# temudschin/xfemm

Hardware: AMD Instinct MI355X
Metric: solved DoF/s (assembly+CG to tol) on 2M-tri magnetostatic (higher is better)
Workload: dtype f64; 1 GPU; configs[2]: synthetic 2000000-tri square-domain magnetostatic, linear mu, tol 1e-08; triangles=2000000, dof_total=1002001, dof_per_gpu=1002001, nnz=7006001, pcg_iters=18, newton_iters=1, pcg=Chronopoulos-Gear + AMG V-cycle, parallelism=single GPU

## Files before the change

### xfemm_amd/csrc/xfk_amg.hip

```cpp
#include <hipcub/hipcub.hpp>

#include <algorithm>
#include <climits>
#include <cmath>
#include <cstdio>
#include <cstdlib>
#include <cstring>
#include <map>
#include <mutex>
#include <vector>

#include "xfk_amg_impl.h"
#include "xfk_comm.h"

namespace xfk {

namespace {



using MisKey = unsigned;
constexpr MisKey kStIn = 2u, kStUnd = 1u;
constexpr MisKey kKeyMask = 0x3FFFFFFFu;

// ... 1253 lines not shown
static int build_col16(hipStream_t st, int n, const int *rowptr, const int *col, long long nnz,
                       DBuf<unsigned short> &c16, DBuf<int> &base)
{
    const int nt = (n + B - 1) / B;
    AMG_CHECK(c16.alloc((size_t)std::max(1LL, nnz)));
    AMG_CHECK(base.alloc((size_t)std::max(1, nt)));
    if (nt > 0) k_tile_col16<B><<<nt, 256, 0, st>>>(n, rowptr, col, c16.p, base.p);
    AMG_CHECK(hipGetLastError());
    return XFK_OK;
}

int Amg::aggregate(hipStream_t s, int l, long long &nc, bool allow_stop)
{
    AmgLevel &A = *L[l];
    const int n = A.n;
    const ColView cv{A.col, A.has16 ? A.a16.p : nullptr, A.has16 ? A.a16b.p : nullptr};
    nc = 0;
    A.nc = 0;
    AMG_CHECK(key.alloc(n));
    AMG_CHECK(t1.alloc(n));
    const std::string lv = g_prof ? "setup L" + std::to_string(l) + " " : std::string();
    if (g_prof) g_prof->begin(lv + "MIS-2 aggregation", 0.0);
    int rounds = 0;
    int *und2 = dev_int.p + 4;
    int *run = dev_int.p + 7;
    AMG_CHECK(act.alloc(n));
    k_mis_init<<<std::max(1, nb(n)), kB, 0, s>>>(n, cnt.p, key.p, und2 + 1, run, act.p);
    AMG_CHECK(flag.alloc((size_t)n + 1));
    AMG_CHECK(cursor.alloc((size_t)n + 1));
    auto hint = mis_hint.find(l);
    const bool spec = !g_prof && !A.dist && hint != mis_hint.end() && cap_hint.count(4 * l) &&
                      def_n + 4 <= kAmgDeferSlots && !env_set("XFK_AMG_DEBUG");
    bool joined = false;
    auto joins_and_p = [&]() { return joins_and_p_impl(s, l); };
    AMG_CHECK(mis_out.alloc(4));
    for (int batch = hint != mis_hint.end() ? std::max(1, hint->second) : 12;; batch = 2) {
        for (int b = 0; b < batch; ++b, ++rounds) {
            int *cur = und2 + (rounds & 1), *prev = und2 + ((rounds + 1) & 1);
            const bool last = b + 1 == batch;
            if (A.nnz > 9LL * n) {
                k_mis_max<4><<<nb(4LL * n), kB, 0, s>>>(n, A.rowptr, cv, sflag.p, key.p, t1.p, prev, cur, run, act.p);
                if (last)
                    k_mis_update<4, true><<<nb(4LL * n), kB, 0, s>>>(n, A.rowptr, cv, sflag.p, t1.p, key.p, prev, cur,
                                                                      flag.p);
                else
                    k_mis_update<4><<<nb(4LL * n), kB, 0, s>>>(n, A.rowptr, cv, sflag.p, t1.p, key.p, prev, cur,
                                                                nullptr);
            } else {
                k_mis_max<1><<<nb(n), kB, 0, s>>>(n, A.rowptr, cv, sflag.p, key.p, t1.p, prev, cur, run, act.p);
                if (last)
                    k_mis_update<1, true><<<nb(n), kB, 0, s>>>(n, A.rowptr, cv, sflag.p, t1.p, key.p, prev, cur,
                                                                flag.p);
                else
                    k_mis_update<1><<<nb(n), kB, 0, s>>>(n, A.rowptr, cv, sflag.p, t1.p, key.p, prev, cur, nullptr);
            }
        }
        int rc = scan_only(*this, s, flag.p, cursor.p, n);
        if (rc != XFK_OK) return rc;
        k_mis_pack<<<1, 64, 0, s>>>(cursor.p + n, und2 + ((rounds - 1) & 1), run, mis_out.p);
        AMG_CHECK(hipMemcpyAsync(host_int + 8, mis_out.p, 3 * sizeof(int), hipMemcpyDeviceToHost, s));
        AMG_CHECK(hipEventRecord(ev_host, s));
        joined = spec;
        if (spec && (rc = joins_and_p()) != XFK_OK) return rc;
        AMG_CHECK(hipEventSynchronize(ev_host));
        if (!host_int[9]) break;
        joined = false;
        if (rounds > 4096) {
            set_error("AMG: MIS-2 aggregation did not terminate");
            return XFK_ERR_NOCONV;
        }
    }
    mis_hint[l] = host_int[10];
    nc = host_int[8];
    stats.mis_rounds[l] = host_int[10];
    int rc = XFK_OK;
    if (allow_stop && (nc == 0 || nc > (long long)(0.9 * n))) {
        nc = 0;
        return XFK_OK;
    }
    if (!joined && (rc = joins_and_p()) != XFK_OK) return rc;
    A.nc = (int)nc;
    if (env_set("XFK_AMG_DEBUG")) std::fprintf(stderr, "[amg] level %d P nnz %lld\n", l, A.pnnz);
    AMG_CHECK(A.rrow.alloc((size_t)nc + 1));
    AMG_CHECK(A.rcol.alloc((size_t)std::max(1LL, A.pnnz)));
    AMG_CHECK(A.rval.alloc((size_t)std::max(1LL, A.pnnz)));
    const bool off = !A.dist && !dist;
    hipStream_t ts = s;
    if (off) {
        if ((rc = sw.init()) != XFK_OK) return rc;
        AMG_CHECK(hipEventRecord(sw.a, s));
        AMG_CHECK(hipStreamWaitEvent(sw.cs, sw.a, 0));
        ts = sw.cs;
        sw_used = true;
    }
    if ((rc = transpose_csr(off ? cnt2 : cnt, off ? cub_tmp2 : cub_tmp, ts, n, (int)nc, A.prow.p, A.pcol.p,
                            A.pval.p, A.rrow.p, A.rcol.p, A.rval.p)) != XFK_OK)
        return rc;
    if (off) {
        AMG_CHECK(hipEventRecord(sw.b, sw.cs));
        rt_pending = true;
    }
    if (l == 0 && A.has16 && (rc = build_col16<256>(ts, (int)nc, A.rrow.p, A.rcol.p, A.pnnz, A.r16, A.r16b)) != XFK_OK)
        return rc;
    if (l == 0 && A.has32 && (rc = to_f32(ts, (int)nc, A.rrow.p, A.pnnz, A.rval.p, A.r32)) != XFK_OK) return rc;
    if (l == 0 && A.has32 && A.dist &&
        ((rc = to_f32(ts, n, A.prow.p, A.pnnz, A.pval.p, A.p32)) != XFK_OK ||
         (rc = build_col16<256>(ts, n, A.prow.p, A.pcol.p, A.pnnz, A.p16, A.p16b)) != XFK_OK))
        return rc;
    if (g_prof) g_prof->end();
    return XFK_OK;
}

int Amg::joins_and_p_impl(hipStream_t s, int l)
{
    AmgLevel &A = *L[l];
    const int n = A.n;
    const ColView cv{A.col, A.has16 ? A.a16.p : nullptr, A.has16 ? A.a16b.p : nullptr};
    const std::string lv = g_prof ? "setup L" + std::to_string(l) + " " : std::string();
    AMG_CHECK(agg1.alloc(n));
    AMG_CHECK(agg.alloc(n));
    const int jg = join_lanes((double)A.nnz / std::max(1, n));
    auto joins = [&](auto g) {
        constexpr int G = decltype(g)::value;
        const int blocks = nb((long long)n * G);
        k_agg_join1<G><<<blocks, kB, 0, s>>>(n, A.rowptr, cv, sflag.p, key.p, cursor.p, agg1.p);
        k_agg_join2<G><<<blocks, kB, 0, s>>>(n, A.rowptr, cv, sflag.p, key.p, agg1.p, agg.p);
        k_agg_join3<G><<<blocks, kB, 0, s>>>(n, A.ncol_lim, A.rowptr, cv, A.val, agg.p, agg1.p);
    };
    if (jg == 8) joins(std::integral_constant<int, 8>{});
    else if (jg == 4) joins(std::integral_constant<int, 4>{});
    else joins(std::integral_constant<int, 1>{});
    std::swap(agg.p, agg1.p);
    std::swap(agg.n, agg1.n);
    if (g_prof) g_prof->end();
    if (env_set("XFK_AMG_DEBUG")) {
        DBuf<int> d;
        AMG_CHECK(d.alloc(3));
        AMG_CHECK(hipMemsetAsync(d.p, 0, 3 * sizeof(int), s));
        k_debug_unagg<<<nb(n), kB, 0, s>>>(n, A.rowptr, A.col, cnt.p, agg.p, d.p);
        int h[3];
        unsigned long long r2[2];
        AMG_CHECK(hipMemcpyAsync(h, d.p, sizeof(h), hipMemcpyDeviceToHost, s));
        AMG_CHECK(hipMemcpyAsync(r2, rho.p + 2 * l, sizeof(r2), hipMemcpyDeviceToHost, s));
        AMG_CHECK(hipStreamSynchronize(s));
        double ra, rf;
        std::memcpy(&ra, &r2[0], 8);
        std::memcpy(&rf, &r2[1], 8);
        std::fprintf(stderr, "[amg] rank %d level %d n %d nnz %lld nc %lld unaggregated: strong %d weak-only %d isolated %d "
                     "rhoA/omega %.4g rhoF %.4g mis_rounds %d\n", dist ? rank : 0, l, n, A.nnz, (long long)host_int[8], h[0], h[1],
                     h[2], ra, rf, host_int[10]);
    }
    SgX XS{A.rowptr, A.col, A.val, A.ncol_lim, sflag.p, dfinv.p, wF.p, cv.c16, cv.cbase};
    SgY YT{nullptr, nullptr, nullptr, agg.p};
    if (g_prof) g_prof->begin(lv + "P = (I - w D^-1 A) P_tent, R = P^T", 0.0);
    return spgemm<true>(*this, s, n, XS, YT, A.prow, A.pcol, A.pval, A.pnnz, 4 * l, !A.dist);
}

int Amg::alloc_vectors()
{
    for (int k = 0; k < nlev; ++k) {
        AmgLevel &A = *L[k];
        const size_t nv = (size_t)std::max(1, std::max(A.n, A.ncol_smooth));
        AMG_CHECK(A.xa.alloc(nv));
        AMG_CHECK(A.xb.alloc(nv));
        AMG_CHECK(A.r.alloc((size_t)std::max(1, A.n)));
        if (k > 0) AMG_CHECK(A.b.alloc((size_t)std::max(1, A.n)));
    }
    return XFK_OK;
}

int Amg::build(hipStream_t s, int l0)
{
    int l = l0;
    for (;; ++l) {
        AmgLevel &A = *L[l];
        const int n = A.n;
        stats.n[l] = n;
        stats.nnz[l] = A.nnz;
        A.nc = 0;
        AMG_CHECK(A.dinv.alloc(n));
        AMG_CHECK(absd.alloc(n));
        AMG_CHECK(dfinv.alloc(n));
        AMG_CHECK(wF.alloc(n));
        AMG_CHECK(cnt.alloc((size_t)n + 1));
        const std::string lv = g_prof ? "setup L" + std::to_string(l) + " " : std::string();
        if (g_prof) g_prof->begin(lv + "diagonal, strength, rho", 0.0);
        k_amg_diag<<<nb(n), kB, 0, s>>>(n, A.rowptr, A.col, A.val, absd.p, A.dinv.p);
        if (n <= dense_max) {
            if (g_prof) g_prof->end();
            dense_coarse = true;
            break;
        }
        A.has16 = l == 0 && !A.dist && !dist && col16 != 0;
        A.has32 = A.has16 && prec32 != 0;
        if (A.has16) {
            int rc0 = build_col16<kCgBlock>(s, n, A.rowptr, A.col, A.nnz, A.a16, A.a16b);
            if (rc0 != XFK_OK) return rc0;
        }
        AMG_CHECK(sflag.alloc((size_t)A.nnz));
        AMG_CHECK(rho_part.alloc(2 * (size_t)nb_str(n)));
        k_amg_strength<<<nb_str(n), kB, 0, s>>>(n, A.ncol_lim, theta_at(l), A.rowptr,
                                                ColView{A.col, A.has16 ? A.a16.p : nullptr, A.has16 ? A.a16b.p : nullptr},
                                                A.val, absd.p, A.dinv.p, sflag.p, cnt.p,
                                                dfinv.p, wF.p, rho_part.p);
        k_max_reduce<<<1, kMaxReduceT, 0, s>>>(nb_str(n), rho_part.p, omega, rho.p + 2 * l);
        if (g_prof) g_prof->end();
        if (trace) {
            int rct = trace_strength(s, l);
            if (rct != XFK_OK) return rct;
        }
        if (l == kAmgMaxLevels - 1) break;
        long long nc = 0;
        int rc = aggregate(s, l, nc, true);
        if (rc != XFK_OK) return rc;
        if (nc == 0) break;
        if (trace && (rc = trace_aggregates(s, l)) != XFK_OK) return rc;
        SgX XA{A.rowptr, A.col, A.val, A.ncol_lim, nullptr, nullptr, nullptr, A.has16 ? A.a16.p : nullptr,
               A.has16 ? A.a16b.p : nullptr};
        SgY YP{A.prow.p, A.pcol.p, A.pval.p, nullptr};
        if (fold_pending) {
            AMG_CHECK(hipStreamWaitEvent(s, sw.c, 0));
            fold_pending = false;
        }
        if (g_prof) g_prof->begin(lv + "SpGEMM A P", 0.0);
        const bool pack = !A.dist && nc < kPackMaxCol && spgemm_pack_on();
        XA.pack = pack;
        rc = spgemm<false>(*this, s, n, XA, YP, A.ftrow, ap_col, ap_val, ap_nnz, 4 * l + 1);
        if (g_prof) g_prof->end();
        if (rc != XFK_OK) return rc;
        if ((int)L.size() <= l + 1) L.emplace_back(new AmgLevel());
        AmgLevel &C = *L[l + 1];
        SgX XR{A.rrow.p, A.rcol.p, A.rval.p, INT_MAX, nullptr, nullptr, nullptr};
        XR.pack = pack;
        SgY YAP{A.ftrow.p, ap_col.p, ap_val.p, nullptr};
        if (rt_pending) {
            AMG_CHECK(hipStreamWaitEvent(s, sw.b, 0));
            rt_pending = false;
        }
        if (g_prof) g_prof->begin(lv + "SpGEMM R (A P)", 0.0);
        rc = spgemm<false>(*this, s, (int)nc, XR, YAP, C.rowptr_o, C.col_o, C.val_o, C.nnz, 4 * l + 2);
        if (g_prof) g_prof->end();
        if (rc != XFK_OK) return rc;
        A.fold = fold_on != 0 && sweeps == 1 && !A.dist;
        A.fold_formed = A.fold;
        if (A.fold) {
            if (g_prof) g_prof->begin(lv + "folded transfer P~ = (I - w D^-1 A) P, R~ = P~^T", 0.0);
            A.fnnz = ap_nnz;
            AMG_CHECK(A.ftrow.alloc((size_t)n + 1));
            AMG_CHECK(A.ftcol.alloc((size_t)std::max(1LL, ap_nnz)));
            AMG_CHECK(A.ftval.alloc((size_t)std::max(1LL, ap_nnz)));
            if (l > 0) {
                AMG_CHECK(A.frrow.alloc((size_t)nc + 1));
                AMG_CHECK(A.frcol.alloc((size_t)std::max(1LL, ap_nnz)));
                AMG_CHECK(A.frval.alloc((size_t)std::max(1LL, ap_nnz)));
            }
            if ((rc = sw.init()) != XFK_OK) return rc;
            AMG_CHECK(hipEventRecord(sw.a, s));
            AMG_CHECK(hipStreamWaitEvent(sw.cs, sw.a, 0));
            hipStream_t fs = sw.cs;
            sw_used = true;
            if (n > 0)
                k_fold_p<<<(int)(((long long)n * kFoldLanes + 255) / 256), 256, 0, fs>>>(
                    n, rho.p + 2 * l, A.dinv.p, A.ftrow.p, ap_col.p, ap_val.p, A.prow.p, A.pcol.p, A.pval.p, A.ftcol.p,
                    A.ftval.p);
            if (l == 0 && A.has16 &&
                (rc = build_col16<kCgBlock>(fs, n, A.ftrow.p, A.ftcol.p, ap_nnz, A.f16, A.f16b)) != XFK_OK)
                return rc;
            if (l == 0 && A.has32 && (rc = to_f32(fs, n, A.ftrow.p, ap_nnz, A.ftval.p, A.f32v)) != XFK_OK) return rc;
            AMG_CHECK(hipEventRecord(sw.c, sw.cs));
            fold_pending = true;
            if (l > 0)
                rc = transpose_csr(cnt2, cub_tmp2, fs, n, (int)nc, A.ftrow.p, A.ftcol.p, A.ftval.p, A.frrow.p,
                                   A.frcol.p, A.frval.p);
            if (rc != XFK_OK) return rc;
            if (def_n > 0 && def_n + 2 <= kAmgDeferSlots) {
                AMG_CHECK(hipMemcpyAsync(def_dev.p + def_n + 1, A.ftrow.p + n, sizeof(int), hipMemcpyDeviceToDevice, s));
                def_target[def_n / 2] = &A.fnnz;
                def_n += 2;
            } else if (def_n > 0) {
                int len = 0;
                AMG_CHECK(hipMemcpyAsync(&len, A.ftrow.p + n, sizeof(int), hipMemcpyDeviceToHost, s));
                AMG_CHECK(hipStreamSynchronize(s));
                A.fnnz = len;
            }
            if (g_prof) g_prof->end();
        }
        C.n = (int)nc;
        C.ncol_lim = (int)nc;
        C.ncol_smooth = (int)nc;
        C.rowptr = C.rowptr_o.p;
        C.col = C.col_o.p;
        C.val = C.val_o.p;
    }
    nlev = l + 1;
    {
        AmgLevel &C = *L[nlev - 1];
        const bool nd_spec = dense_coarse && !g_prof && def_n > 0 && nlev - 1 > l0 &&
                             C.n >= 8 * kBj && nd_key_n == C.n && C.col == C.col_o.p &&
                             (size_t)nd_key_nnz <= C.col_o.n && !env_set("XFK_NO_ND");
        if (nd_spec) {
            AMG_CHECK(mis_out.alloc(4));
            AMG_CHECK(hipMemsetAsync(mis_out.p + 3, 0, sizeof(int), s));
            const int nt = (int)std::max((long long)C.n + 1, nd_key_nnz);
            k_pattern_diff<<<nb(nt), kB, 0, s>>>(C.n, C.rowptr, C.col, nd_key_dev.p, (int)nd_key_nnz, mis_out.p + 3);
            AMG_CHECK(hipMemcpyAsync(host_int + 11, mis_out.p + 3, sizeof(int), hipMemcpyDeviceToHost, s));
        }
// ... 758 lines not shown
```

### xfemm_amd/csrc/xfk_amg_spgemm.hip

```cpp
#include <hipcub/hipcub.hpp>

#include <algorithm>
#include <climits>

#include "xfk_amg_impl.h"

namespace xfk {

namespace {


constexpr int kSgMax = 512;

constexpr int ilog2(int v) { return v <= 1 ? 0 : 1 + ilog2(v >> 1); }

template <bool FILL, bool PMODE, int CAP>
__global__ void __launch_bounds__(64) k_spgemm(int nrows, SgX X, SgY Y, int *__restrict__ cnt_out,
                                               const int *__restrict__ crow, int *__restrict__ ccol,
                                               double *__restrict__ cval, int *overflow)
{
    constexpr int kSgHash = 2 * CAP;
    constexpr int kHashShift = 32 - ilog2(kSgHash);
    __shared__ int hk[kSgHash];
    __shared__ int hr[FILL ? kSgHash : 1];
// ... 57 lines not shown
                    if (f != 0 && Y.agg[k] >= 0) {
                        ys = k;
                        len = 1;
                        xv = (f == 2) ? 1.0 - omega : -omega * dfi * X.val[e];
                    }
                } else {
                    ys = Y.rowptr[k];
                    len = Y.rowptr[k + 1] - ys;
                    xv = X.val[e];
                }
            }
        }
        int incl = len;
#pragma unroll
        for (int off = 1; off < 64; off <<= 1) {
            const int t = __shfl_up(incl, off, 64);
            if (lane >= off) incl += t;
        }
        const int total = __shfl(incl, 63, 64);
        c_off[lane] = incl - len;
        c_ys[lane] = ys;
        c_xv[lane] = xv;
        __syncthreads();
        return total;
    };
    auto product = [&](int p, int &key, double &v) {
        int lo = 0, hi = 63;
        while (lo < hi) {
            const int mid = (lo + hi + 1) >> 1;
            if (c_off[mid] <= p) lo = mid;
            else hi = mid - 1;
        }
        if (PMODE) {
            key = Y.agg[c_ys[lo]];
            v = c_xv[lo];
        } else {
            const int q = c_ys[lo] + (p - c_off[lo]);
            key = Y.col[q];
            if (FILL) v = c_xv[lo] * Y.val[q];
        }
    };

    for (int e0 = xs; e0 < xe; e0 += 64) {
        const int total = stage(e0);
        for (int p = lane; p < total; p += 64) {
            int key;
            double v;
            product(p, key, v);
            insert(key);
        }
        __syncthreads();
    }
    if (!FILL) {
        if (lane == 0) {
            cnt_out[row] = s_cnt;
            if (s_ovf || s_cnt > CAP) atomicOr(overflow, 1);
        }
        return;
    }
    for (int t = lane; t < kSgHash; t += 64)
        if (hk[t] != -1) {
            const int m = atomicAdd(&s_m, 1);
            if (m < CAP) {
                lst[m] = hk[t];
                lslot[m] = t;
            }
        }
    __syncthreads();
    const int cnt = min(s_m, CAP);
    const int cb = crow[row];
    for (int m = lane; m < cnt; m += 64) {
        const int key = lst[m];
        int rank = 0;
        for (int q = 0; q < cnt; ++q) rank += lst[q] < key;
        hr[lslot[m]] = rank;
        ccol[cb + rank] = key;
        acc[rank] = 0.0;
    }
    __syncthreads();
    const int4 *r4 = reinterpret_cast<const int4 *>(s_rank);
    for (int e0 = xs; e0 < xe; e0 += 64) {
        const int total = stage(e0);
        for (int p0 = 0; p0 < total; p0 += 64) {
            const int p = p0 + lane;
            int rank = -1;
            double v = 0.0;
            if (p < total) {
                int key;
                product(p, key, v);
                const int h = lookup(key);
                rank = (h >= 0) ? hr[h] : -1;
            }
            s_rank[lane] = rank;
            s_val[lane] = v;
            __syncthreads();
            if (rank >= 0) {
                bool leader = true;
                double sum = 0.0;
#pragma unroll
                for (int m4 = 0; m4 < 16; ++m4) {
                    const int4 q = r4[m4];
                    const int m = 4 * m4;
                    if (q.x == rank) { leader &= (m < lane) ? false : true; sum += s_val[m]; }
                    if (q.y == rank) { leader &= (m + 1 < lane) ? false : true; sum += s_val[m + 1]; }
                    if (q.z == rank) { leader &= (m + 2 < lane) ? false : true; sum += s_val[m + 2]; }
                    if (q.w == rank) { leader &= (m + 3 < lane) ? false : true; sum += s_val[m + 3]; }
                }
                if (leader) acc[rank] += sum;
            }
            __syncthreads();
        }
    }
    for (int m = lane; m < cnt; m += 64) cval[cb + m] = acc[m];
}

template <bool PMODE>
__global__ void k_spgemm_nprod(int nrows, SgX X, SgY Y, int *__restrict__ nprod)
{
    const int row = blockIdx.x * blockDim.x + threadIdx.x;
    if (row >= nrows) return;
    int c = 0;
    for (int e = X.rowptr[row]; e < X.rowptr[row + 1]; ++e) {
        const int k = X.col[e];
        if (k >= X.col_lim) continue;
        if (PMODE) c += (X.mask[e] != 0 && Y.agg[k] >= 0);
        else c += Y.rowptr[k + 1] - Y.rowptr[k];
    }
    nprod[row] = c;
}


__device__ __forceinline__ void wave_lds_sync()
{
    __builtin_amdgcn_fence(__ATOMIC_RELEASE, "wavefront");
    __builtin_amdgcn_wave_barrier();
    __builtin_amdgcn_fence(__ATOMIC_ACQUIRE, "wavefront");
}

__device__ __forceinline__ unsigned xor_lanes(unsigned w, int lm)
{
    const int x = (int)w;
    switch (lm) {
    case 1: return (unsigned)__builtin_amdgcn_update_dpp(x, x, 0xB1, 0xF, 0xF, false);
    case 2: return (unsigned)__builtin_amdgcn_update_dpp(x, x, 0x4E, 0xF, 0xF, false);
    case 4: {
        const int t = __builtin_amdgcn_update_dpp(x, x, 0x104, 0xF, 0x5, false);
        return (unsigned)__builtin_amdgcn_update_dpp(t, x, 0x114, 0xF, 0xA, false);
    }
    case 8: return (unsigned)__builtin_amdgcn_update_dpp(x, x, 0x128, 0xF, 0xF, false);
    default: return (unsigned)__shfl_xor(x, lm, 64);
    }
}

template <bool PMODE, int G, int CAP, bool PACK = false>
__global__ void __launch_bounds__(64) k_spgemm_sort(int nrows, SgX X, SgY Y, int *__restrict__ cnt_out,
                                                    int *__restrict__ pcol, double *__restrict__ pval, int *ovf,
                                                    int *need, int *__restrict__ slab_n)
{
    constexpr int W = 64 / G;
    constexpr int S = CAP / G;
    static_assert(S >= 1 && S * G == CAP, "CAP must be a multiple of G");
    __shared__ int pk_all[W][CAP];
    __shared__ double pv_all[W][CAP];
    const int g = threadIdx.x / G, l = threadIdx.x % G;
    const int row = blockIdx.x * W + g;
    int *pk = pk_all[g];
    double *pv = pv_all[g];
    const bool live = row < nrows;
    int np = 0;
    if (live) {
        const int xs = X.rowptr[row], xe = X.rowptr[row + 1];
        const ColView xc{X.col, X.c16, X.cbase};
        const int cb = xc.base(row);
        double omega = 0.0, dfi = 0.0;
        if (PMODE) {
            omega = X.wF[row];
            dfi = X.dfinv[row];
        }
        for (int e0 = xs; e0 < xe; e0 += G) {
            const int e = e0 + l;
            int len = 0, ys = 0;
            double xv = 0.0;
            if (e < xe) {
                const int k = xc.at(cb, e);
                if (k < X.col_lim) {
                    if (PMODE) {
                        const unsigned char f = X.mask[e];
                        if (f != 0 && Y.agg[k] >= 0) {
                            ys = Y.agg[k];
                            len = 1;
                            xv = (f == 2) ? 1.0 - omega : -omega * dfi * X.val[e];
                        }
                    } else {
                        ys = Y.rowptr[k];
                        len = Y.rowptr[k + 1] - ys;
                        xv = X.val[e];
                    }
                }
            }
            int incl = len;
#pragma unroll
            for (int off = 1; off < G; off <<= 1) {
                const int t = __shfl_up(incl, off, G);
                if (l >= off) incl += t;
            }
            const int total = __shfl(incl, G - 1, G);
            const int o = np + incl - len;
            if (PMODE) {
                if (len && o < CAP) {
                    pk[o] = ys;
                    pv[o] = xv;
                }
            } else {
                constexpr int U = CAP >= 128 ? 8 : 4;
                int yc[U];
                double yv[U];
#pragma unroll
                for (int q = 0; q < U; ++q)
                    if (q < len) {
                        yc[q] = Y.col[ys + q];
                        yv[q] = Y.val[ys + q];
                    }
#pragma unroll
                for (int q = 0; q < U; ++q)
                    if (q < len && o + q < CAP) {
                        pk[o + q] = yc[q];
                        pv[o + q] = xv * yv[q];
                    }
                for (int q = U; q < len && o + q < CAP; ++q) {
                    pk[o + q] = Y.col[ys + q];
                    pv[o + q] = xv * Y.val[ys + q];
                }
            }
            np += total;
        }
        if (need && np > CAP / 2 && l == 0 && *(volatile int *)need == 0) *need = 1;
        if (np > CAP) {
            if (l == 0) *ovf = 1;
            np = CAP;
        }
    }
    wave_lds_sync();
    int key[S];
    double val[S];
    if constexpr (PACK) {
        constexpr int B = ilog2(CAP);
        unsigned w[S];
#pragma unroll
        for (int s = 0; s < S; ++s) {
            const int v = l * S + s;
            w[s] = v < np ? ((unsigned)pk[v] << B) | (unsigned)v : ~0u;
        }
#pragma unroll
        for (int k = 2; k <= CAP; k <<= 1) {
#pragma unroll
            for (int j = k >> 1; j > 0; j >>= 1) {
                if (j < S) {
#pragma unroll
                    for (int s = 0; s < S; ++s) {
                        const int t = s ^ j;
                        if (t > s) {
                            const bool up = ((l * S + s) & k) == 0;
                            const unsigned a = w[s] >> B, b = w[t] >> B;
                            if ((a > b) == up && a != b) {
                                const unsigned tw = w[s];
                                w[s] = w[t];
                                w[t] = tw;
                            }
                        }
                    }
                } else {
                    const int lm = j / S;
                    const bool lower = (l & lm) == 0;
#pragma unroll
                    for (int s = 0; s < S; ++s) {
                        const unsigned ow = xor_lanes(w[s], lm);
                        const unsigned a = w[s] >> B, b = ow >> B;
                        const bool up = ((l * S + s) & k) == 0;
                        const bool take = (lower == up) ? (b < a) : (b > a);
                        if (take) w[s] = ow;
                    }
                }
            }
        }
#pragma unroll
        for (int s = 0; s < S; ++s) {
            const bool real = w[s] != ~0u;
            key[s] = real ? (int)(w[s] >> B) : INT_MAX;
            val[s] = real ? pv[w[s] & (unsigned)(CAP - 1)] : 0.0;
        }
    } else {
#pragma unroll
        for (int s = 0; s < S; ++s) {
            const int v = l * S + s;
            key[s] = v < np ? pk[v] : INT_MAX;
            val[s] = v < np ? pv[v] : 0.0;
        }
#pragma unroll
        for (int k = 2; k <= CAP; k <<= 1) {
#pragma unroll
            for (int j = k >> 1; j > 0; j >>= 1) {
                if (j < S) {
#pragma unroll
                    for (int s = 0; s < S; ++s) {
                        const int t = s ^ j;
                        if (t > s) {
                            const bool up = ((l * S + s) & k) == 0;
                            if ((key[s] > key[t]) == up && key[s] != key[t]) {
                                const int tk = key[s];
                                key[s] = key[t];
                                key[t] = tk;
                                const double tv = val[s];
                                val[s] = val[t];
                                val[t] = tv;
                            }
                        }
                    }
                } else {
                    const int lm = j / S;
                    const bool lower = (l & lm) == 0;
#pragma unroll
                    for (int s = 0; s < S; ++s) {
                        const int ok = __shfl_xor(key[s], lm, G);
                        const double ov = __shfl_xor(val[s], lm, G);
                        const bool up = ((l * S + s) & k) == 0;
                        const bool take = (lower == up) ? (ok < key[s]) : (ok > key[s]);
                        if (take) {
                            key[s] = ok;
                            val[s] = ov;
                        }
                    }
                }
            }
        }
    }
    const int prev_last = __shfl_up(key[S - 1], 1, G);
    int head[S], nh = 0;
    double run[S];
#pragma unroll
    for (int s = 0; s < S; ++s) {
        const int pk_ = s > 0 ? key[s - 1] : (l > 0 ? prev_last : -1);
        head[s] = (key[s] != INT_MAX && key[s] != pk_) ? 1 : 0;
        run[s] = (s > 0 && !head[s]) ? run[s - 1] + val[s] : val[s];
        nh += head[s];
    }
    int seg_open = 1;
#pragma unroll
    for (int s = 0; s < S; ++s) seg_open &= !head[s];
    double carry = run[S - 1];
    int hpre = nh;
    int open = seg_open;
#pragma unroll
    for (int off = 1; off < G; off <<= 1) {
        const double oc = __shfl_up(carry, off, G);
        const int oo = __shfl_up(open, off, G);
        const int oh = __shfl_up(hpre, off, G);
        if (l >= off) {
            if (open) carry = oc + carry;
            open = open && oo;
            hpre += oh;
        }
    }
    double cin = __shfl_up(carry, 1, G);
    int hin = __shfl_up(hpre, 1, G);
    if (l == 0) {
        cin = 0.0;
        hin = 0;
    }
    const int cnt = __shfl(hpre, G - 1, G);
    int upto = cnt;
#pragma unroll
    for (int off = G; off < 64; off <<= 1) {
        const int t = __shfl_up(upto, off, 64);
        if ((int)threadIdx.x >= off) upto += t;
    }
    if (slab_n && threadIdx.x == 63) slab_n[blockIdx.x] = upto;
    if (!live) return;
    const size_t base = slab_n ? (size_t)blockIdx.x * (W * CAP) + (upto - cnt) : (size_t)row * CAP;
    int h = hin;
#pragma unroll
    for (int s = 0; s < S; ++s) {
        bool lead = true;
#pragma unroll
        for (int q = 0; q <= s; ++q) lead = lead && !head[q];
        const double tot = lead ? cin + run[s] : run[s];
        h += head[s];
        const int nk = s + 1 < S ? key[s + 1] : __shfl_down(key[0], 1, G);
        const bool tail = key[s] != INT_MAX && (nk != key[s] || (s + 1 == S && l == G - 1));
        if (tail) {
            pcol[base + h - 1] = key[s];
            pval[base + h - 1] = tot;
        }
    }
    if (l == 0) cnt_out[row] = cnt;
}

template <int L>
__global__ void k_spgemm_compact(int nrows, int cap, const int *__restrict__ crow, const int *__restrict__ pcol,
                                 const double *__restrict__ pval, int *__restrict__ ccol, double *__restrict__ cval,
                                 int *nnz_out)
{
    const long long t = blockIdx.x * (long long)blockDim.x + threadIdx.x;
    if (t == 0 && nnz_out) *nnz_out = crow[nrows];
    const int row = (int)(t / L), l = (int)(t % L);
    if (row >= nrows) return;
    const int b = crow[row], n = crow[row + 1] - b;
    for (int m = l; m < n; m += L) {
        ccol[b + m] = pcol[(size_t)row * cap + m];
        cval[b + m] = pval[(size_t)row * cap + m];
    }
}

constexpr int kSlabLanes = 16;
__global__ void k_spgemm_compact_slab(int nrows, int nslab, int W, int stride, const int *__restrict__ crow,
                                      const int *__restrict__ slab_n, const int *__restrict__ pcol,
                                      const double *__restrict__ pval, int *__restrict__ ccol,
                                      double *__restrict__ cval, int *nnz_out)
{
    const long long t = blockIdx.x * (long long)blockDim.x + threadIdx.x;
    if (t == 0 && nnz_out) *nnz_out = crow[nrows];
    const int b = (int)(t / kSlabLanes), l = (int)(t % kSlabLanes);
    if (b >= nslab) return;
    const int d = crow[b * W], n = slab_n[b];
    const size_t src = (size_t)b * stride;
    for (int m = l; m < n; m += kSlabLanes) {
        ccol[d + m] = pcol[src + m];
        cval[d + m] = pval[src + m];
    }
}

static bool spgemm_slab_on()
{
    return env_int("XFK_SPGEMM_SLAB", 1) != 0;
}
static int sort_rows_per_wave(int cap) { return cap == 16 ? 16 : cap <= 64 ? 8 : cap == 128 ? 4 : 2; }

void launch_compact(hipStream_t s, int nrows, int cap, const int *crow, const int *slab_n, const int *pc,
                    const double *pv, int *ccol, double *cval, int *nnz_out)
{
    if (slab_n) {
        const int W = sort_rows_per_wave(cap), nslab = (nrows + W - 1) / W;
        k_spgemm_compact_slab<<<(unsigned)(((long long)nslab * kSlabLanes + kB - 1) / kB), kB, 0, s>>>(
            nrows, nslab, W, W * cap, crow, slab_n, pc, pv, ccol, cval, nnz_out);
    } else if (cap <= 16)
        k_spgemm_compact<4><<<(unsigned)(((long long)nrows * 4 + kB - 1) / kB), kB, 0, s>>>(nrows, cap, crow, pc, pv,
                                                                                             ccol, cval, nnz_out);
    else if (cap <= 32)
        k_spgemm_compact<8><<<(unsigned)(((long long)nrows * 8 + kB - 1) / kB), kB, 0, s>>>(nrows, cap, crow, pc, pv,
                                                                                             ccol, cval, nnz_out);
    else
        k_spgemm_compact<16><<<(unsigned)(((long long)nrows * 16 + kB - 1) / kB), kB, 0, s>>>(nrows, cap, crow, pc,
                                                                                               pv, ccol, cval, nnz_out);
}

}

template <bool PMODE>
int spgemm(Amg &M, hipStream_t s, int nrows, const SgX &X, const SgY &Y, DBuf<int> &crow, DBuf<int> &ccol,
           DBuf<double> &cval, long long &cnnz, int key, bool defer)
{
    AMG_CHECK(M.cnt.alloc((size_t)nrows + 1 + ((size_t)nrows + 1) / 2));
    AMG_CHECK(crow.alloc((size_t)nrows + 1));
    int *slab_n = spgemm_slab_on() ? M.cnt.p + nrows + 1 : nullptr;
    int *sovf = M.dev_int.p + 6;
    auto launch_sort = [&](int cap, int *ovf, int *need = nullptr) {
        int *pc = M.pad_col.p;
        double *pv = M.pad_val.p;
        if (nrows > 0) {
#define XFK_SORT(GG, CC, WW)                                                       \
    (X.pack ? k_spgemm_sort<PMODE, GG, CC, !PMODE> : k_spgemm_sort<PMODE, GG, CC>) \
        <<<(nrows + WW - 1) / WW, 64, 0, s>>>(nrows, X, Y, M.cnt.p, pc, pv, ovf, need, slab_n)
            if (cap == 16) XFK_SORT(4, 16, 16);
            else if (cap == 32) XFK_SORT(8, 32, 8);
            else if (cap == 64) XFK_SORT(8, 64, 8);
            else if (cap == 128) XFK_SORT(16, 128, 4);
            else XFK_SORT(32, 256, 2);
#undef XFK_SORT
        }
    };
    auto sort_pass = [&](int cap, bool &overflow) -> int {
        AMG_CHECK(M.pad_col.alloc((size_t)nrows * cap));
        AMG_CHECK(M.pad_val.alloc((size_t)nrows * cap));
        AMG_CHECK(hipMemsetAsync(sovf, 0, sizeof(int), s));
        launch_sort(cap, sovf);
        AMG_CHECK(hipMemcpyAsync(M.host_int + 4, sovf, sizeof(int), hipMemcpyDeviceToHost, s));
        int rc = scan_total(M, s, M.cnt.p, crow.p, nrows, cnnz);
        if (rc != XFK_OK) return rc;
        overflow = M.host_int[4] != 0;
        if (overflow) return XFK_OK;
        AMG_CHECK(ccol.alloc((size_t)std::max(1LL, cnnz)));
        AMG_CHECK(cval.alloc((size_t)std::max(1LL, cnnz)));
        if (nrows > 0)
            launch_compact(s, nrows, cap, crow.p, slab_n, M.pad_col.p, M.pad_val.p, ccol.p, cval.p, nullptr);
        return XFK_OK;
    };
    auto deferred_pass = [&](int cap, bool verify = false) -> int {
        int *slot = M.def_dev.p + M.def_n;
        int *need = (verify && cap > 16) ? M.def_dev.p + kAmgDeferSlots + M.def_n / 2 : nullptr;
        M.def_verify[M.def_n / 2] = need ? cap : 0;
        AMG_CHECK(M.pad_col.alloc((size_t)nrows * cap));
        AMG_CHECK(M.pad_val.alloc((size_t)nrows * cap));
        AMG_CHECK(ccol.alloc((size_t)std::max(1LL, (long long)nrows * cap)));
        AMG_CHECK(cval.alloc((size_t)std::max(1LL, (long long)nrows * cap)));
        launch_sort(cap, slot, need);
        int rc = scan_only(M, s, M.cnt.p, crow.p, nrows);
        if (rc != XFK_OK) return rc;
        if (nrows > 0)
            launch_compact(s, nrows, cap, crow.p, slab_n, M.pad_col.p, M.pad_val.p, ccol.p, cval.p, slot + 1);
        else
            AMG_CHECK(hipMemsetAsync(slot + 1, 0, sizeof(int), s));
        M.def_target[M.def_n / 2] = &cnnz;
        M.def_n += 2;
        cnnz = (long long)nrows * cap;
        return XFK_OK;
    };
    if (key >= 0) {
        auto hint = M.cap_hint.find(key);
        if (hint != M.cap_hint.end()) {
            if (defer && M.def_n + 2 <= kAmgDeferSlots) return deferred_pass(hint->second, M.foreign);
            if (M.foreign) {
                M.cap_hint.erase(hint);
                hint = M.cap_hint.end();
            }
        }
        if (hint != M.cap_hint.end()) {
            bool overflow = false;
            int rc = sort_pass(hint->second, overflow);
            if (rc != XFK_OK || !overflow) return rc;
            M.cap_hint.erase(hint);
        }
    }
    int maxprod = 0;
    if (nrows > 0) {
        k_spgemm_nprod<PMODE><<<nb(nrows), kB, 0, s>>>(nrows, X, Y, M.cnt.p);
        size_t bytes = 0;
        AMG_CHECK(hipcub::DeviceReduce::Max(nullptr, bytes, M.cnt.p, M.dev_int.p + 3, nrows, s));
        AMG_CHECK(M.cub_tmp.alloc(bytes ? bytes : 1));
        AMG_CHECK(hipcub::DeviceReduce::Max(M.cub_tmp.p, bytes, M.cnt.p, M.dev_int.p + 3, nrows, s));
        int rc = read_flag(M, s, 3, maxprod);
        if (rc != XFK_OK) return rc;
    }
    if (maxprod <= kSortCap) {
        const int cap = maxprod <= 16 ? 16 : maxprod <= 32 ? 32 : maxprod <= 64 ? 64 : maxprod <= 128 ? 128 : 256;
        int rc = XFK_OK;
        if (defer && key >= 0 && M.def_n + 2 <= kAmgDeferSlots) {
            rc = deferred_pass(cap);
        } else {
            bool overflow = false;
            rc = sort_pass(cap, overflow);
            if (rc == XFK_OK && overflow) {
                set_error("AMG: internal SpGEMM capacity error");
                return XFK_ERR_HIP;
            }
        }
        if (rc != XFK_OK) return rc;
        if (key >= 0) {
            const bool small = env_set("XFK_AMG_TEST_SMALL_HINT");
            M.cap_hint[key] = small ? 16 : cap;
        }
        return XFK_OK;
    }
    AMG_CHECK(hipMemsetAsync(M.dev_int.p + 2, 0, 2 * sizeof(int), s));
    if (nrows > 0)
        k_spgemm<false, PMODE, kSgMax><<<nrows, 64, 0, s>>>(nrows, X, Y, M.cnt.p, nullptr, nullptr, nullptr,
                                                            M.dev_int.p + 2);
    if (nrows > 0) {
        size_t bytes = 0;
        AMG_CHECK(hipcub::DeviceReduce::Max(nullptr, bytes, M.cnt.p, M.dev_int.p + 3, nrows, s));
        AMG_CHECK(M.cub_tmp.alloc(bytes ? bytes : 1));
        AMG_CHECK(hipcub::DeviceReduce::Max(M.cub_tmp.p, bytes, M.cnt.p, M.dev_int.p + 3, nrows, s));
    }
    AMG_CHECK(hipMemcpyAsync(M.host_int + 2, M.dev_int.p + 2, 2 * sizeof(int), hipMemcpyDeviceToHost, s));
    int rc = scan_total(M, s, M.cnt.p, crow.p, nrows, cnnz);
    if (rc != XFK_OK) return rc;
    const int ovf = M.host_int[2], maxrow = M.host_int[3];
    if (ovf) {
        set_error("AMG: a SpGEMM row exceeds the LDS hash capacity");
        return XFK_ERR_UNSUPPORTED;
    }
    AMG_CHECK(ccol.alloc((size_t)std::max(1LL, cnnz)));
    AMG_CHECK(cval.alloc((size_t)std::max(1LL, cnnz)));
    if (nrows > 0) {
        int *of = M.dev_int.p + 2;
        if (maxrow <= 32)
            k_spgemm<true, PMODE, 32><<<nrows, 64, 0, s>>>(nrows, X, Y, nullptr, crow.p, ccol.p, cval.p, of);
        else if (maxrow <= 128)
            k_spgemm<true, PMODE, 128><<<nrows, 64, 0, s>>>(nrows, X, Y, nullptr, crow.p, ccol.p, cval.p, of);
        else
            k_spgemm<true, PMODE, kSgMax><<<nrows, 64, 0, s>>>(nrows, X, Y, nullptr, crow.p, ccol.p, cval.p, of);
    }
    return XFK_OK;
}

template int spgemm<false>(Amg &, hipStream_t, int, const SgX &, const SgY &, DBuf<int> &, DBuf<int> &,
                           DBuf<double> &, long long &, int, bool);
template int spgemm<true>(Amg &, hipStream_t, int, const SgX &, const SgY &, DBuf<int> &, DBuf<int> &,
                          DBuf<double> &, long long &, int, bool);

}

hipError_t xfk::warm_module_amg_spgemm()
{
    hipFuncAttributes a;
    return hipFuncGetAttributes(&a, reinterpret_cast<const void *>(&k_spgemm_compact_slab));
}
```

Baseline: 192.7 million DoF/s.

## Scan per-slab counts in SpGEMM sort and derive row offsets in compaction

The sorted SpGEMM kernel now uses DPP lane moves instead of generic shuffles for its small-group prefix scans, and computes each row's offset within its wave slab. The global scan runs over per-slab totals instead of per-row counts, and the slab compaction kernel writes crow from slab offsets plus row offsets. Packed-column mode is also enabled for the prolongator product. This targets AMG setup cost (scan length and shuffle latency), at the cost of more complex index bookkeeping and extra scratch space.

```diff
diff --git a/xfemm_amd/csrc/xfk_amg.hip b/xfemm_amd/csrc/xfk_amg.hip
--- a/xfemm_amd/csrc/xfk_amg.hip
+++ b/xfemm_amd/csrc/xfk_amg.hip
@@ -1429,6 +1429,7 @@
     }
     SgX XS{A.rowptr, A.col, A.val, A.ncol_lim, sflag.p, dfinv.p, wF.p, cv.c16, cv.cbase};
     SgY YT{nullptr, nullptr, nullptr, agg.p};
+    XS.pack = !A.dist && n < kPackMaxCol && spgemm_pack_on();
     if (g_prof) g_prof->begin(lv + "P = (I - w D^-1 A) P_tent, R = P^T", 0.0);
     return spgemm<true>(*this, s, n, XS, YT, A.prow, A.pcol, A.pval, A.pnnz, 4 * l, !A.dist);
 }
diff --git a/xfemm_amd/csrc/xfk_amg_spgemm.hip b/xfemm_amd/csrc/xfk_amg_spgemm.hip
--- a/xfemm_amd/csrc/xfk_amg_spgemm.hip
+++ b/xfemm_amd/csrc/xfk_amg_spgemm.hip
@@ -233,6 +233,35 @@
     }
 }
 
+template <int G>
+__device__ __forceinline__ int up_lanes(int x, int d)
+{
+    if constexpr (G <= 16) {
+        switch (d) {
+        case 1: return __builtin_amdgcn_update_dpp(x, x, 0x111, 0xF, 0xF, false);
+        case 2: return __builtin_amdgcn_update_dpp(x, x, 0x112, 0xF, 0xF, false);
+        case 4: return __builtin_amdgcn_update_dpp(x, x, 0x114, 0xF, 0xF, false);
+        case 8: return __builtin_amdgcn_update_dpp(x, x, 0x118, 0xF, 0xF, false);
+        default: break;
+        }
+    }
+    return __shfl_up(x, d, G);
+}
+template <int G>
+__device__ __forceinline__ double up_lanes(double x, int d)
+{
+    if constexpr (G <= 16)
+        return __hiloint2double(up_lanes<G>(__double2hiint(x), d), up_lanes<G>(__double2loint(x), d));
+    else
+        return __shfl_up(x, d, G);
+}
+template <int G>
+__device__ __forceinline__ int down_lane(int x)
+{
+    if constexpr (G <= 16) return __builtin_amdgcn_update_dpp(x, x, 0x101, 0xF, 0xF, false);
+    else return __shfl_down(x, 1, G);
+}
+
 template <bool PMODE, int G, int CAP, bool PACK = false>
 __global__ void __launch_bounds__(64) k_spgemm_sort(int nrows, SgX X, SgY Y, int *__restrict__ cnt_out,
                                                     int *__restrict__ pcol, double *__restrict__ pval, int *ovf,
@@ -282,7 +311,7 @@
             int incl = len;
 #pragma unroll
             for (int off = 1; off < G; off <<= 1) {
-                const int t = __shfl_up(incl, off, G);
+                const int t = up_lanes<G>(incl, off);
                 if (l >= off) incl += t;
             }
             const int total = __shfl(incl, G - 1, G);
@@ -415,7 +444,7 @@
             }
         }
     }
-    const int prev_last = __shfl_up(key[S - 1], 1, G);
+    const int prev_last = up_lanes<G>(key[S - 1], 1);
     int head[S], nh = 0;
     double run[S];
 #pragma unroll
@@ -433,27 +462,36 @@
     int open = seg_open;
 #pragma unroll
     for (int off = 1; off < G; off <<= 1) {
-        const double oc = __shfl_up(carry, off, G);
-        const int oo = __shfl_up(open, off, G);
-        const int oh = __shfl_up(hpre, off, G);
+        const double oc = up_lanes<G>(carry, off);
+        const int oo = up_lanes<G>(open, off);
+        const int oh = up_lanes<G>(hpre, off);
         if (l >= off) {
             if (open) carry = oc + carry;
             open = open && oo;
             hpre += oh;
         }
     }
-    double cin = __shfl_up(carry, 1, G);
-    int hin = __shfl_up(hpre, 1, G);
+    double cin = up_lanes<G>(carry, 1);
+    int hin = up_lanes<G>(hpre, 1);
     if (l == 0) {
         cin = 0.0;
         hin = 0;
     }
     const int cnt = __shfl(hpre, G - 1, G);
     int upto = cnt;
-#pragma unroll
-    for (int off = G; off < 64; off <<= 1) {
-        const int t = __shfl_up(upto, off, 64);
-        if ((int)threadIdx.x >= off) upto += t;
+    if constexpr (G <= 16) {
+#pragma unroll
+        for (int off = G; off < 16; off <<= 1) {
+            const int t = up_lanes<16>(upto, off);
+            if ((int)(threadIdx.x & 15) >= off) upto += t;
+        }
+        const int r0 = __builtin_amdgcn_readlane(upto, 15), r1 = __builtin_amdgcn_readlane(upto, 31),
+                  r2 = __builtin_amdgcn_readlane(upto, 47);
+        const int rw = threadIdx.x >> 4;
+        upto += (rw > 0 ? r0 : 0) + (rw > 1 ? r1 : 0) + (rw > 2 ? r2 : 0);
+    } else {
+        const int r0 = __builtin_amdgcn_readlane(cnt, 31);
+        if (threadIdx.x >= 32) upto += r0;
     }
     if (slab_n && threadIdx.x == 63) slab_n[blockIdx.x] = upto;
     if (!live) return;
@@ -466,14 +504,14 @@
         for (int q = 0; q <= s; ++q) lead = lead && !head[q];
         const double tot = lead ? cin + run[s] : run[s];
         h += head[s];
-        const int nk = s + 1 < S ? key[s + 1] : __shfl_down(key[0], 1, G);
+        const int nk = s + 1 < S ? key[s + 1] : down_lane<G>(key[0]);
         const bool tail = key[s] != INT_MAX && (nk != key[s] || (s + 1 == S && l == G - 1));
         if (tail) {
             pcol[base + h - 1] = key[s];
             pval[base + h - 1] = tot;
         }
     }
-    if (l == 0) cnt_out[row] = cnt;
+    if (l == 0) cnt_out[row] = slab_n ? upto - cnt : cnt;
 }
 
 template <int L>
@@ -493,16 +531,23 @@
 }
 
 constexpr int kSlabLanes = 16;
-__global__ void k_spgemm_compact_slab(int nrows, int nslab, int W, int stride, const int *__restrict__ crow,
-                                      const int *__restrict__ slab_n, const int *__restrict__ pcol,
-                                      const double *__restrict__ pval, int *__restrict__ ccol,
-                                      double *__restrict__ cval, int *nnz_out)
+__global__ void k_spgemm_compact_slab(int nrows, int nslab, int W, int stride, const int *__restrict__ slab_off,
+                                      const int *__restrict__ slab_n, const int *__restrict__ row_off,
+                                      const int *__restrict__ pcol, const double *__restrict__ pval,
+                                      int *__restrict__ crow, int *__restrict__ ccol, double *__restrict__ cval,
+                                      int *nnz_out)
 {
     const long long t = blockIdx.x * (long long)blockDim.x + threadIdx.x;
-    if (t == 0 && nnz_out) *nnz_out = crow[nrows];
+    if (t == 0) {
+        const int total = slab_off[nslab];
+        crow[nrows] = total;
+        if (nnz_out) *nnz_out = total;
+    }
     const int b = (int)(t / kSlabLanes), l = (int)(t % kSlabLanes);
     if (b >= nslab) return;
-    const int d = crow[b * W], n = slab_n[b];
+    const int d = slab_off[b], n = slab_n[b];
+    const int row = b * W + l;
+    if (l < W && row < nrows) crow[row] = d + row_off[row];
     const size_t src = (size_t)b * stride;
     for (int m = l; m < n; m += kSlabLanes) {
         ccol[d + m] = pcol[src + m];
@@ -516,13 +561,14 @@
 }
 static int sort_rows_per_wave(int cap) { return cap == 16 ? 16 : cap <= 64 ? 8 : cap == 128 ? 4 : 2; }
 
-void launch_compact(hipStream_t s, int nrows, int cap, const int *crow, const int *slab_n, const int *pc,
-                    const double *pv, int *ccol, double *cval, int *nnz_out)
+static_assert(kSlabLanes >= 16, "a slab's lanes write its rows' crow entries: one lane per row, W <= 16");
+void launch_compact(hipStream_t s, int nrows, int cap, int *crow, const int *slab_n, const int *slab_off,
+                    const int *row_off, const int *pc, const double *pv, int *ccol, double *cval, int *nnz_out)
 {
     if (slab_n) {
         const int W = sort_rows_per_wave(cap), nslab = (nrows + W - 1) / W;
         k_spgemm_compact_slab<<<(unsigned)(((long long)nslab * kSlabLanes + kB - 1) / kB), kB, 0, s>>>(
-            nrows, nslab, W, W * cap, crow, slab_n, pc, pv, ccol, cval, nnz_out);
+            nrows, nslab, W, W * cap, slab_off, slab_n, row_off, pc, pv, crow, ccol, cval, nnz_out);
     } else if (cap <= 16)
         k_spgemm_compact<4><<<(unsigned)(((long long)nrows * 4 + kB - 1) / kB), kB, 0, s>>>(nrows, cap, crow, pc, pv,
                                                                                              ccol, cval, nnz_out);
@@ -540,16 +586,21 @@
 int spgemm(Amg &M, hipStream_t s, int nrows, const SgX &X, const SgY &Y, DBuf<int> &crow, DBuf<int> &ccol,
            DBuf<double> &cval, long long &cnnz, int key, bool defer)
 {
-    AMG_CHECK(M.cnt.alloc((size_t)nrows + 1 + ((size_t)nrows + 1) / 2));
+    const size_t slab_max = ((size_t)nrows + 1) / 2 + 1;
+    AMG_CHECK(M.cnt.alloc((size_t)nrows + 1 + 2 * slab_max + 1));
     AMG_CHECK(crow.alloc((size_t)nrows + 1));
-    int *slab_n = spgemm_slab_on() ? M.cnt.p + nrows + 1 : nullptr;
+    int *slab_n = (nrows > 0 && spgemm_slab_on()) ? M.cnt.p + nrows + 1 : nullptr;
+    int *slab_off = slab_n ? slab_n + slab_max : nullptr;
+    auto nscan = [&](int cap) { return slab_n ? (nrows + sort_rows_per_wave(cap) - 1) / sort_rows_per_wave(cap) : nrows; };
+    const int *scan_in = slab_n ? slab_n : M.cnt.p;
+    int *scan_out = slab_n ? slab_off : crow.p;
     int *sovf = M.dev_int.p + 6;
     auto launch_sort = [&](int cap, int *ovf, int *need = nullptr) {
         int *pc = M.pad_col.p;
         double *pv = M.pad_val.p;
         if (nrows > 0) {
-#define XFK_SORT(GG, CC, WW)                                                       \
-    (X.pack ? k_spgemm_sort<PMODE, GG, CC, !PMODE> : k_spgemm_sort<PMODE, GG, CC>) \
+#define XFK_SORT(GG, CC, WW)                                                     \
+    (X.pack ? k_spgemm_sort<PMODE, GG, CC, true> : k_spgemm_sort<PMODE, GG, CC>) \
         <<<(nrows + WW - 1) / WW, 64, 0, s>>>(nrows, X, Y, M.cnt.p, pc, pv, ovf, need, slab_n)
             if (cap == 16) XFK_SORT(4, 16, 16);
             else if (cap == 32) XFK_SORT(8, 32, 8);
@@ -565,14 +616,15 @@
         AMG_CHECK(hipMemsetAsync(sovf, 0, sizeof(int), s));
         launch_sort(cap, sovf);
         AMG_CHECK(hipMemcpyAsync(M.host_int + 4, sovf, sizeof(int), hipMemcpyDeviceToHost, s));
-        int rc = scan_total(M, s, M.cnt.p, crow.p, nrows, cnnz);
+        int rc = scan_total(M, s, scan_in, scan_out, nscan(cap), cnnz);
         if (rc != XFK_OK) return rc;
         overflow = M.host_int[4] != 0;
         if (overflow) return XFK_OK;
         AMG_CHECK(ccol.alloc((size_t)std::max(1LL, cnnz)));
         AMG_CHECK(cval.alloc((size_t)std::max(1LL, cnnz)));
         if (nrows > 0)
-            launch_compact(s, nrows, cap, crow.p, slab_n, M.pad_col.p, M.pad_val.p, ccol.p, cval.p, nullptr);
+            launch_compact(s, nrows, cap, crow.p, slab_n, slab_off, M.cnt.p, M.pad_col.p, M.pad_val.p, ccol.p, cval.p,
+                           nullptr);
         return XFK_OK;
     };
     auto deferred_pass = [&](int cap, bool verify = false) -> int {
@@ -584,10 +636,11 @@
         AMG_CHECK(ccol.alloc((size_t)std::max(1LL, (long long)nrows * cap)));
         AMG_CHECK(cval.alloc((size_t)std::max(1LL, (long long)nrows * cap)));
         launch_sort(cap, slot, need);
-        int rc = scan_only(M, s, M.cnt.p, crow.p, nrows);
+        int rc = scan_only(M, s, scan_in, scan_out, nscan(cap));
         if (rc != XFK_OK) return rc;
         if (nrows > 0)
-            launch_compact(s, nrows, cap, crow.p, slab_n, M.pad_col.p, M.pad_val.p, ccol.p, cval.p, slot + 1);
+            launch_compact(s, nrows, cap, crow.p, slab_n, slab_off, M.cnt.p, M.pad_col.p, M.pad_val.p, ccol.p, cval.p,
+                           slot + 1);
         else
             AMG_CHECK(hipMemsetAsync(slot + 1, 0, sizeof(int), s));
         M.def_target[M.def_n / 2] = &cnnz;
```

Result: faster. 194.8 million DoF/s, median of 6 (+1.1%).
